# djeday123/kaldi-fp16

Measured on AMD Instinct MI355X. Metric: frames/sec CNN-TDNN fwd+bwd, 40-dim×1500-frame egs, 1/2/4/8 MI355X, higher is better.
Workload: dtype fp16

## Files before the change

### include/kf_ops.h

```cpp
#ifndef KALDI_FP16_AMD_KF_OPS_H
#define KALDI_FP16_AMD_KF_OPS_H

#include <stddef.h>
#include <stdint.h>

#ifdef __cplusplus
extern "C" {
#endif

#define KF_MAX_PARTS 9
#define KF_ZERO 0
#define KF_CLAMP 1

typedef struct {
    const void *base;
    long long ld;
    int nrows, ncols;
    int kcontig;
    int nparts, part_width;
    int T, hout, hsrc, hmul, hdiv, tpolicy;
    int dt[KF_MAX_PARTS];
    int dh[KF_MAX_PARTS];
    int edge_t[KF_MAX_PARTS];
    int edge_row[KF_MAX_PARTS];
// ... 149 lines not shown
                void *scratch);
long long kf_ng_state_scratch_bytes(const KfNgPre *pres, int npre);
int kf_ng_state(const KfNgPre *pres, const KfNgPre *pres_dev, int npre, const KfNgOpts *opts, int update,
                float *w32, void *w16, double *sc, const float *stat, void *scratch, float *report);

#define KF_DROP_MAX 32
typedef struct KfDropLayer {
    float *mask;
    long long ld;
    int dim;
    int ordinal;
    float p;
    int reserved;
} KfDropLayer;
int kf_dropout_masks(int n, const KfDropLayer *layers, int B, unsigned long long seed, long long step);
int kf_row_seg(int32_t *row_seg, const int *dev_seq_off, int B, int T, int tc0, int tc);

int kf_specaug_rows(int32_t *row_band, const int *dev_seq_off, int B, int T, int dim, int max_bins, float z,
                    int max_zeroed, int max_kept, unsigned ordinal, unsigned long long seed, long long step);
int kf_specaug_apply(const void *x, long long ldx, void *y, long long ldy, long long rows, int dim,
                     const int32_t *row_band);

int kf_bn_train_stats(const void *r, long long ld, int rows, int D, float eps, float target_rms, float *mean,
                      float *var, float *scale, float *shift, double *acc_count, double *acc_sum, double *acc_sumsq);
int kf_bn_train_apply(const void *r, long long ld, int rows, int D, const float *scale, const float *shift,
                      const float *drop, long long ld_drop, const int32_t *row_seg, const void *resid, long long ldr,
                      float alpha, void *out, long long ldo);
int kf_bn_train_bwd_stats(const void *g, long long ldg, const void *r, long long ldr, int rows, int D,
                          const float *scale, const float *shift, float target_rms, const float *drop,
                          long long ld_drop, const int32_t *row_seg, float *a, float *b);
int kf_bn_train_bwd_apply(const void *g, long long ldg, const void *r, long long ldr, int rows, int D,
                          const float *scale, const float *shift, float target_rms, const float *a, const float *b,
                          const float *drop, long long ld_drop, const int32_t *row_seg, const uint8_t *mask,
                          long long ld_mask, void *dz, long long lddz);

int kf_gather_rows(void *dst, const void *src, long long row_bytes, int T, int tc0, int tc);
int kf_scatter_rows(void *dst, const void *src, long long row_bytes, int T, int tc0, int tc);
int kf_scatter_rows_from(void *dst, const void *src, long long row_bytes, int T, int tc0, int tc, int r0);
int kf_rows_sum_list(void *edge, const void *src, long long ld, const int *rows, int n, int cols);
const char *kf_layers_last_error(void);

enum { KF_CM_ONEBYTE_COLHDR = 1, KF_CM_TWOBYTE = 2, KF_CM_ONEBYTE = 3, KF_CM_FLOAT = 4 };
typedef struct {
    int format, rows, cols, out_row;
    float min_value, range;
    long long payload_off;
} KfCmDesc;
int kf_cm_expand(const KfCmDesc *dev_desc, int nmat, int max_rows, int max_cols,
                 const void *dev_blob, void *dev_out, int ldo);
int kf_cm_expand_host(const KfCmDesc *desc, int nmat, int max_rows, int max_cols,
                      const void *blob, size_t blob_bytes, void *dev_out, int ldo);

typedef struct {
    const void *proj;
    long long ldp;
    int T, num_heads, key_dim, value_dim, context, num_left, stride;
    float key_scale;
} KfAttention;
int kf_attention_forward(const KfAttention *a, void *out, long long ldo, uint8_t *mask, const float *scale,
                         const float *shift);
int kf_attention_backward(const KfAttention *a, const void *dz, long long ldz, void *dproj, float *scratch);

int kf_combine_feature_maps(const void *a, long long lda, const void *b, long long ldb, const int *dev_seq_off,
                            int B, void *out, long long ldo, int T, int height, int nf1, int nf2);
int kf_combine_feature_maps_backward(const void *dy, long long ldy, const int *dev_seq_off, int B, void *db,
                                     long long ldb, int height, int nf1, int nf2);
int kf_im2col_small(const void *x, long long ldx, int T, int hin, int hout, int sub, int fin, int ntaps,
                    const int *dt, const int *dh, void *P, int kp);
int kf_col2im_small(const void *dP, int T, int hin, int hout, int sub, int fin, int ntaps, const int *dt,
                    const int *dh, int kp, void *dx, long long ldx);
int kf_rows_gemm(const void *x, long long ldx, const void *W, long long ldw, void *y, long long ldy, int R, int K,
                 int N);
int kf_rows_wgrad(const void *x, long long ldx, const void *g, long long ldg, float *dW, long long ldd, int R, int M,
                  int N);
int kf_scale_cols(const void *x, long long ldx, const float *scale, void *y, long long ldy, int rows, int cols);

void kf_prof_enable(int on);
int kf_prof_reserve(int n);
int kf_prof_collect(int cls, long long *count, double *ms, double *flops);
int kf_prof_collect2(int cls, long long *count, double *ms, double *flops, double *bytes);
void kf_prof_reset(void);

void kf_gemm_debug_kil(int on);
#define KF_TRANSPOSE_MAX 48
int kf_transpose_batch(int n, const void *const *src, void *const *dst, const int *M, const int *N);
void kf_halo_trace(unsigned long long *buf, int at);
int kf_halo_debug_last(int *out, int n);
void kf_gemm_trace(unsigned long long *buf, int at, int blk);

const char *kf_last_error(void);
void kf_clear_error(void);
int kf_prof_records(int max, int *cls, float *ms, double *flops, int *mnkt);

int kf_take_pending(const char *where);
const char *kf_pending_log(void);
void kf_pending_clear(void);
int kf_peek_error(void);
int kf_debug_spin(void *stream, long long cycles);

#ifdef __cplusplus
}
#endif
#endif
```

### kaldi-fp16_amd/csrc/conv_halo.hip

```cpp
#include "gemm_kernel.h"

__device__ __forceinline__ int halo_off(int R, int c) {
    return (R >> 3) * 1024 + 256 * (c >> 1) + 16 * ((c + 2 * R) & 15);
}
struct HaloArgs {
    const h16 *x;
    long long ld;
    int T, hout, hmul, hsrc, pw, pad, hpe, hpos, nf, dtmin;
    int ntaps, nch;
    int ts, toff;
    int rows;
    int npieces;
    int slice;
    int halo_bytes;
    int nbuf;
    int ctap[KF_MAX_PARTS];
    int bshift[KF_MAX_PARTS];
    unsigned mhpos;
    unsigned long long *trace;
};


template <int BM, int BN, int WM, int WN, bool BKC, int BMODE, bool BROW, int ST>
__global__ __launch_bounds__(64 * WM * WN, 1) void conv_halo_kernel(int M, int N, OpD B, KfEpilogue E,
                                                                    HaloArgs H, int n_mtiles,
                                                                    int n_ntiles) {
    constexpr int NW = WM * WN;
    constexpr int WTM = BM / WM, WTN = BN / WN;
    constexpr int TM = WTM / 16, TN = WTN / 16;
    constexpr int B_STAGE = BN * BK * 2;
    constexpr int NWB = NW / 2;
    using SB = Stager<BKC, BN, BMODE, NWB>;
    static_assert(SB::EVEN, "uniform B loads per B wave");
    static_assert(ST == 2, "the split-wave waits are written for a two-stage B ring");
    extern __shared__ __attribute__((aligned(16))) char dsm[];
    char *bring = dsm + H.nbuf * H.halo_bytes;

    const int tid = threadIdx.x, lane = tid & 63;
    const int wave = __builtin_amdgcn_readfirstlane(tid >> 6);
    const int wm = wave / WN, wn = wave % WN;

    const int ntiles = n_mtiles * n_ntiles;
    int tile = blockIdx.x;
    if (ntiles >= 8) {
        const int q = ntiles / 8, rmd = ntiles % 8, xcd = tile % 8, loc = tile / 8;
        tile = (xcd < rmd ? xcd * (q + 1) : rmd * (q + 1) + (xcd - rmd) * q) + loc;
    }
    const int mt = tile / n_ntiles, nt = tile - mt * n_ntiles;
    const int m0 = mt * BM, n0 = nt * BN;
    const int tbase = H.ts * (m0 / H.hout) + H.toff + H.dtmin;

    const bool bwave = wave < NWB;
    SB sb;
    if (bwave) sb.init(B, n0, wave, lane);
    const Rsrc rx = make_rsrc(H.x), rb = make_rsrc(B.base);
    const int K = H.ntaps * H.pw;

    auto halo_issue = [&](int c, int img, int q0, int q1, int w0, int nw) {
        char *dst = dsm + img * H.halo_bytes;
        const int slot = lane & 15, kc = 2 * (lane >> 4) + (slot & 1), r = ((slot - kc) & 15) >> 1;
        if (wave < w0) return;
        for (int q = q0 + wave - w0; q < q1; q += nw) {
            const int R = 8 * q + r;
            unsigned voff = BAD;
            if (R < H.rows) {
                const int f = (int)__umulhi((unsigned)R, H.mhpos), pos = R - f * H.hpos;
                const int par = pos >= H.hpe ? 1 : 0, idx = pos - par * H.hpe;
                const int sh = idx * H.hmul + par - H.pad, t = tbase + f;
                if ((unsigned)t < (unsigned)H.T && (unsigned)sh < (unsigned)H.hsrc)
                    voff = (unsigned)(((long long)t * H.ld + (long long)sh * H.pw + c * BK + kc * 8) * 2);
            }
            lds_dma<16>(rx, dst + q * 1024, voff);
        }
    };

    int rb0[TM];
    static_for<TM>([&](auto I) {
        const int r = wm * WTM + I * 16 + (lane & 15);
        const int m = min(m0 + r, M - 1);
        const int t = m / H.hout, h = m - t * H.hout;
        rb0[I] = (H.ts * t + H.toff - tbase + H.dtmin) * H.hpos + h;
    });

    float4v acc[TM][TN];
    static_for<TM>([&](auto I) {
        static_for<TN>([&](auto J) { acc[I][J] = float4v{0.f, 0.f, 0.f, 0.f}; });
    });
// ... 220 lines not shown
```

### kaldi-fp16_amd/csrc/gemm_common.h

```cpp
#pragma once
#include <utility>

#include "kf_common.h"
#include "../../include/kf_ops.h"

struct OpD {
    const h16 *base;
    long long ld;
    int nrows, ncols;
    int nparts, pw;
    int T, hout, hsrc, hmul, hshift;
    int tclamp, simple, p64;
    unsigned inv_hout;
    unsigned ldb, pwb;
    int edges;
    int dt[KF_MAX_PARTS], dh[KF_MAX_PARTS], et[KF_MAX_PARTS], er[KF_MAX_PARTS];
    const uint8_t *sc;
    unsigned lds;
    int pw8;
    const uint8_t *mk;
    unsigned mlim;
    int tmul, t0;
};

#include <utility>
template <typename F, int... Is>
__device__ __forceinline__ void static_for_impl(F &&f, std::integer_sequence<int, Is...>) {
    (f(std::integral_constant<int, Is>{}), ...);
}
template <int N, typename F>
__device__ __forceinline__ void static_for(F &&f) {
    static_for_impl(f, std::make_integer_sequence<int, N>{});
}

template <typename T>
__device__ __forceinline__ T sel9(const T (&a)[KF_MAX_PARTS], int p, int nparts) {
    if (nparts <= 2) return p ? a[1] : a[0];
    T v = a[0];
#pragma unroll
    for (int i = 1; i < KF_MAX_PARTS; ++i)
        if (p == i) v = a[i];
    return v;
}

__device__ __forceinline__ long long op_off(const OpD &d, int t, int h, int kk, int dtp, int dhp,
                                            int etp, int erp) {
    int st;
    if (t == etp) {
        st = erp;
    } else {
        st = t + dtp;
        if (d.tclamp) st = min(max(st, 0), d.T - 1);
        else if ((unsigned)st >= (unsigned)d.T) return -1;
    }
    int sh = h * d.hmul + dhp;
    if (d.hshift) {
        if (sh & ((1 << d.hshift) - 1)) return -1;
        sh >>= d.hshift;
    }
    if ((unsigned)sh >= (unsigned)d.hsrc) return -1;
    return (long long)st * d.ld + (long long)sh * d.pw + kk;
}

constexpr int BK = 64;
__device__ __forceinline__ int kc_off(int r, int c) { return r * 128 + 16 * (c ^ ((r >> 1) & 7)); }
template <int W>
__device__ __forceinline__ int mn_swz(int r) {
    if constexpr (W % 128 == 0) return ((r & 3) << 2) ^ (((r >> 3) & 1) << 4);
    else if constexpr (W % 64 == 0) return ((r & 2) << 1) ^ (((r >> 3) & 1) << 3);
    else if constexpr (W % 32 == 0) return ((r >> 3) & 1) << 2;
    else return 0;
}
template <int W>
__device__ __forceinline__ int mn_off(int r, int u) {
    return r * (W * 2) + 8 * (u ^ mn_swz<W>(r));
}

typedef __attribute__((address_space(3))) short4v lds_s4;
typedef int v4i_t __attribute__((ext_vector_type(4)));

template <bool KC, int W>
__device__ __forceinline__ half8 load_frag(const char *tile, int idx0, int s, int lane) {
    if constexpr (KC) {
        const int r = idx0 + (lane & 15);
        const int c = s * 4 + (lane >> 4);
        return *reinterpret_cast<const half8 *>(tile + kc_off(r, c));
    } else {
        const int q = (lane & 15) >> 2, p = lane & 3, g = lane >> 4;
        const int r0 = s * 32 + 8 * g + q;
        const int u = (idx0 >> 2) + p;
        short4v lo = __builtin_amdgcn_ds_read_tr16_b64_v4i16((lds_s4 *)(tile + mn_off<W>(r0, u)));
        short4v hi =
            __builtin_amdgcn_ds_read_tr16_b64_v4i16((lds_s4 *)(tile + mn_off<W>(r0 + 4, u)));
        typedef short short8v __attribute__((ext_vector_type(8)));
        short8v v = __builtin_shufflevector(lo, hi, 0, 1, 2, 3, 4, 5, 6, 7);
        return __builtin_bit_cast(half8, v);
    }
}

enum { OP_SIMPLE = 0, OP_P2 = 1, OP_GEN = 2 };
constexpr int OP_MASKED = 8;
constexpr int EPI_DROP = 16;
constexpr unsigned BAD = 0xFFFFFFFFu;

typedef unsigned Rsrc __attribute__((ext_vector_type(4)));
__device__ __forceinline__ Rsrc make_rsrc(const void *base) {
    const unsigned long long b = (unsigned long long)base;
    return Rsrc{(unsigned)__builtin_amdgcn_readfirstlane((unsigned)b),
                (unsigned)__builtin_amdgcn_readfirstlane((unsigned)(b >> 32)) & 0xFFFFu, 0xFFFFFFFFu, 0x00020000u};
}

template <int BYTES>
__device__ __forceinline__ void lds_dma(Rsrc rs, const void *lds_dst, unsigned voff) {
    const unsigned m0v = (unsigned)__builtin_amdgcn_readfirstlane((unsigned)(uintptr_t)lds_dst);
    unsigned keep;
    if constexpr (BYTES == 16)
        asm volatile("s_mov_b32 %0, m0\n\ts_mov_b32 m0, %3\n\ts_nop 0\n\tbuffer_load_dwordx4 %1, %2, 0 offen lds\n\t"
                     "s_mov_b32 m0, %0"
                     : "=&s"(keep)
                     : "v"(voff), "s"(rs), "s"(m0v)
                     : "memory");
    else
        asm volatile("s_mov_b32 %0, m0\n\ts_mov_b32 m0, %3\n\ts_nop 0\n\tbuffer_load_dword %1, %2, 0 offen lds\n\t"
                     "s_mov_b32 m0, %0"
                     : "=&s"(keep)
                     : "v"(voff), "s"(rs), "s"(m0v)
                     : "memory");
}

__device__ __forceinline__ unsigned op_boff(const OpD &d, int t, int h, int kk, int dtp, int dhp,
                                            int etp, int erp) {
    const long long off = op_off(d, t, h, kk, dtp, dhp, etp, erp);
    return off < 0 ? BAD : (unsigned)(off * 2);
}

template <bool KC, int TR, int MODE, int NW, bool MK = false>
struct Stager {
    static constexpr int NP = TR / 8;
    static constexpr int NC = (NP + NW - 1) / NW;
    static constexpr bool EVEN = NC * NW == NP;
    static_assert(NP * 8 == TR, "tile rows must be a multiple of 8");
    unsigned o0[NC];
    unsigned o1[MODE == OP_P2 && KC ? NC : 1];
    int th[MODE == OP_GEN ? NC : 1];
    int dt1[!KC && MODE != OP_SIMPLE ? NC : 1];
    unsigned mbv[MK ? NC : 1];
    int curp;

// ... 278 lines not shown
```

### kaldi-fp16_amd/csrc/gemm_fused.hip

```cpp
#include "gemm_fused.h"

static int g_kil = 1;
extern "C" void kf_gemm_debug_kil(int on) { g_kil = on != 0; }

static int fused_impl(int M, int N, int K, const KfOperand *A, const KfOperand *B, const KfEpilogue *epi,
                      const WgradArgs *edge);
extern "C" int kf_gemm_fused(int M, int N, int K, const KfOperand *A, const KfOperand *B,
                             const KfEpilogue *epi) {
    return fused_impl(M, N, K, A, B, epi, nullptr);
}
extern "C" int kf_gemm_fused_edge(int M, int N, int K, const KfOperand *A, const KfOperand *B,
                                  const KfEpilogue *epi, void *edge_out, const void *x0, const void *x1,
                                  const void *W, int cols) {
    if (!edge_out || !x0 || !x1 || !W || cols <= 0 || cols % 8 || ((uintptr_t)x0 | (uintptr_t)x1 | (uintptr_t)W) & 15 ||
        A->fmt != KF_FMT_MXFP8 || M <= 0) {
        kf_report_error("kf_gemm_fused_edge: an MXFP8 product with M > 0, an edge row and 16-byte aligned fp16 "
                        "operands, cols %% 8 == 0 (cols=%d)", cols);
        return -1;
    }
    WgradArgs g{};
    g.eo = (h16 *)edge_out;
    g.ex0 = (const h16 *)x0;
    g.ex1 = (const h16 *)x1;
    g.ew = (const h16 *)W;
// ... 34 lines not shown
        return -1;
    }
    WgradArgs G{nullptr, nullptr, 0, 0, g_kil};
    if (edge) {
        G.eo = edge->eo;
        G.ex0 = edge->ex0;
        G.ex1 = edge->ex1;
        G.ew = edge->ew;
        G.ecols = edge->ecols;
    }
    const int am = op_mode(a), bm = op_mode(b);
    const bool f8 = A->fmt == KF_FMT_MXFP8;
    if (f8 != (B->fmt == KF_FMT_MXFP8)) {
        kf_report_error("kf_gemm_fused: both operands must be MXFP8, or neither");
        return -1;
    }
    if (E.row_group && (f8 || a.mk || b.mk)) {
        kf_report_error("kf_gemm_fused: grouped output rows (row_group) need an fp16 conv input gradient");
        return -1;
    }
    if (E.drop) {
        if (!E.row_seg || (E.scale != nullptr) == (E.out2 != nullptr)) {
            kf_report_error("kf_gemm_fused: drop needs row_seg and exactly one of scale (forward) and out2 (input "
                            "gradient)");
            return -1;
        }
        if (E.row_group || E.out8 || E.beta != 0.f || f8 || a.mk || b.mk || edge || am == OP_GEN || bm == OP_GEN) {
            kf_report_error("kf_gemm_fused: drop does not go with row_group, out8, beta, MXFP8, masked or conv operands");
            return -1;
        }
        if (E.ld_drop < N || E.ld_drop % 8 || ((uintptr_t)E.drop & 15) || ((uintptr_t)E.row_seg & 3)) {
            kf_report_error("kf_gemm_fused: drop needs ld_drop >= N, ld_drop %% 8 == 0 and a 16-byte aligned table "
                            "(ld_drop=%lld N=%d)", E.ld_drop, N);
            return -1;
        }
    }
    if (f8) {
        if (K % 128 || am == OP_GEN || a.edges || bm != OP_SIMPLE) {
            kf_report_error("kf_gemm_fused: MXFP8 needs K %% 128 == 0, a plain or time-spliced A and a "
                            "plain B (K=%d)", K);
            return -1;
        }
        const int K2 = K / 2;
        if (N % 160 == 0 && N <= 320 && !E.out8) {
            if (am == OP_SIMPLE)
                return launch<384, 160, 4, 2, true, true, false, 2, OP_SIMPLE, OP_SIMPLE, 1>(M, N, K2, a, b, E, G, 1);
            return launch<384, 160, 4, 2, true, true, false, 2, OP_P2, OP_SIMPLE, 1>(M, N, K2, a, b, E, G, 1);
        }
        if (N >= 256) {
            if (am == OP_SIMPLE)
                return launch<256, 256, 2, 4, true, true, false, 2, OP_SIMPLE, OP_SIMPLE, 1>(M, N, K2, a, b, E, G, 1);
            return launch<256, 256, 2, 4, true, true, false, 2, OP_P2, OP_SIMPLE, 1>(M, N, K2, a, b, E, G, 1);
        }
        if (am == OP_SIMPLE)
            return launch<128, 128, 2, 2, true, true, false, 2, OP_SIMPLE, OP_SIMPLE, 1>(M, N, K2, a, b, E, G, 1);
        return launch<128, 128, 2, 2, true, true, false, 2, OP_P2, OP_SIMPLE, 1>(M, N, K2, a, b, E, G, 1);
    }
    if (a.mk || b.mk) {
        if (!b.mk && B->kcontig && !E.out8 && ((am == OP_P2 && bm == OP_P2) || (am == OP_SIMPLE && bm == OP_SIMPLE))) {
            const int mt = N % 160 == 0 && N <= 320 ? 5 : N <= 64 ? 2 : 0;
#define KF_MASKED(AM_, BM_)                                                                                    \
    do {                                                                                                       \
        if (mt == 5) return launch<384, 160, 4, 2, true, true, false, 2, AM_ | OP_MASKED, BM_>(M, N, K, a, b, E, G, 1); \
        if (mt == 2) return launch<256, 64, 4, 1, true, true, false, 2, AM_ | OP_MASKED, BM_>(M, N, K, a, b, E, G, 1);  \
        return launch<128, 128, 2, 2, true, true, false, 2, AM_ | OP_MASKED, BM_>(M, N, K, a, b, E, G, 1);               \
    } while (0)
            if (am == OP_P2) KF_MASKED(OP_P2, OP_P2);
            KF_MASKED(OP_SIMPLE, OP_SIMPLE);
#undef KF_MASKED
        }
        kf_report_error("kf_gemm_fused: a masked operand must be A (plain or two-part time splice, with a "
                        "k-contiguous B of the same kind, no MXFP8 copy) (M=%d N=%d K=%d)", M, N, K);
        return -1;
    }
    if (!E.drop) {
        const int hr = conv_halo_try(M, N, K, a, b, bm, B->kcontig != 0, E);
        if (hr != 0) return hr < 0 ? -1 : 0;
    }
    if (a.tmul > 1 || a.t0 || b.tmul > 1 || b.t0 || E.row_group) {
        kf_report_error("kf_gemm_fused: time-strided rows (tmul / t0) and grouped output rows (row_group) need a "
                        "conv on the halo kernel (M=%d N=%d K=%d)", M, N, K);
        return -1;
    }
    int tile = 0;
    if (N % 160 == 0 && N <= 320 && !E.out8) tile = 5;
    else if (N <= 64) tile = 2;
    else if (N >= 256) tile = 6;
    if (tile == 6 && K <= 640 && N % 192 == 0 && !E.out8) tile = 7;
    if (tile == 5 && (long long)((M + 383) / 384) * ((N + 159) / 160) < 192) tile = 8;
    if (!B->kcontig) return fused_mn(tile, am, bm, M, N, K, a, b, E, G);
    if (E.drop) {
        if (am == OP_SIMPLE && bm == OP_SIMPLE) return fused_tile_drop<true, OP_SIMPLE, OP_SIMPLE>(tile, M, N, K, a, b, E, G);
        if (am == OP_P2 && bm == OP_SIMPLE) return fused_tile_drop<true, OP_P2, OP_SIMPLE>(tile, M, N, K, a, b, E, G);
        if (am == OP_P2 && bm == OP_P2) return fused_tile_drop<true, OP_P2, OP_P2>(tile, M, N, K, a, b, E, G);
        kf_report_error("kf_gemm_fused: drop with a plain A needs a plain B (M=%d N=%d K=%d)", M, N, K);
        return -1;
    }
    if (am == OP_SIMPLE && bm == OP_SIMPLE) return fused_tile<true, OP_SIMPLE, OP_SIMPLE>(tile, M, N, K, a, b, E, G);
    if (am == OP_P2 && bm == OP_SIMPLE) return fused_tile<true, OP_P2, OP_SIMPLE>(tile, M, N, K, a, b, E, G);
    if (am == OP_P2 && bm == OP_P2) return fused_tile<true, OP_P2, OP_P2>(tile, M, N, K, a, b, E, G);
    return fused_tile<true, OP_GEN, OP_GEN>(tile, M, N, K, a, b, E, G);
}
```

### kaldi-fp16_amd/csrc/gemm_host.h

```cpp
#pragma once
#include <algorithm>

#include "gemm_common.h"

double kf_gemm_alg_bytes(const OpD &a, const OpD &b, const KfEpilogue &E, long long M, long long N);

int kf_conv_wgrad_halo_try(int M, int N, int K, const OpD &a, const OpD &b, float *dW, long long ldw,
                           float *bias_grad, int accumulate);
constexpr int KF_HALO_DBG_N = 16;
int *kf_halo_dbg_begin(int kind);

void kf_wgrad_reduce(const float *slab, const float *bias_slab, int splits, int M, int N, float *dW,
                     long long ldw, float *bias_grad, int accumulate, const float *cs = nullptr);

#pragma GCC visibility push(hidden)
bool to_dev(const KfOperand &d, OpD &o, const char *name);
double op_src_bytes(const OpD &o, int f8);
double epi_bytes(const KfEpilogue &E, long long M, long long N);
unsigned long long *kf_gemm_trace_take(int *blk);
int conv_halo_try(int M, int N, int K, const OpD &a, const OpD &b, int bm, bool bkc, const KfEpilogue &E);
#pragma GCC visibility pop

static inline int op_mode(const OpD &o) {
    if (o.simple) return OP_SIMPLE;
    if (o.nparts <= 2 && o.hout == 1 && o.hmul == 0 && o.hshift == 0) return OP_P2;
    return OP_GEN;
}
static inline bool mn_gen_ok(const OpD &o, const char *name) {
    if (op_mode(o) == OP_GEN && o.edges) {
        kf_report_error("operand %s: edge rows need a time-only (<= 2 part) reduction-major operand", name);
        return false;
    }
    return true;
}

static inline KfOperand plain_operand(const void *p, long long ld, int rows, int cols, int kcontig) {
    KfOperand d;
    memset(&d, 0, sizeof(d));
    d.base = p;
    d.ld = ld;
    d.nrows = rows;
    d.ncols = cols;
    d.kcontig = kcontig;
    d.nparts = 1;
    d.part_width = cols;
    d.T = rows;
    d.hout = 1;
    d.hsrc = 1;
    d.hmul = 0;
    d.hdiv = 1;
    d.tpolicy = KF_ZERO;
    for (int i = 0; i < KF_MAX_PARTS; ++i) d.edge_t[i] = -1;
    return d;
}

struct TapGeom {
    int dtmin, dtmax;
    int pad;
    int hpe;
};
static inline TapGeom tap_geometry(const OpD &a) {
    int dtmin = 1 << 20, dtmax = -(1 << 20), dhmin = 1 << 20, dhmax = -(1 << 20);
    for (int p = 0; p < a.nparts; ++p) {
        dtmin = std::min(dtmin, a.dt[p]);
        dtmax = std::max(dtmax, a.dt[p]);
        dhmin = std::min(dhmin, a.dh[p]);
        dhmax = std::max(dhmax, a.dh[p]);
    }
    TapGeom g{dtmin, dtmax, std::max(0, -dhmin), 0};
    const int maxshp = (a.hout - 1) * a.hmul + dhmax + g.pad;
    const int HP = std::max(a.hsrc + g.pad, maxshp + 1);
    g.hpe = (HP + a.hmul - 1) / a.hmul;
    return g;
}
static inline void tap_rows(const OpD &a, const TapGeom &g, int hpe, int *ctap) {
    for (int p = 0; p < a.nparts; ++p) {
        const int x = a.dh[p] + g.pad;
        ctap[p] = (a.dt[p] - g.dtmin) * hpe * a.hmul + (x % a.hmul) * hpe + x / a.hmul;
    }
}
```

### kaldi-fp16_amd/python/kfp16/__init__.py

```python
from __future__ import annotations

import ctypes as C
import os

import numpy as np

_HERE = os.path.dirname(os.path.abspath(__file__))
LIBDIR = os.environ.get("KFP16_LIBDIR") or os.path.normpath(os.path.join(_HERE, "..", "..", "lib"))
INCDIR = os.path.normpath(os.path.join(_HERE, "..", "..", "..", "include"))


class KfError(RuntimeError):
    pass


def _load(name):
    path = os.path.join(LIBDIR, name)
    if not os.path.exists(path):
        raise ImportError(
            f"kfp16: {path} is missing — build the HIP libraries first "
            "(python -c 'import __graft_entry__ as g; g.build()'); there is no CPU fallback")
    if os.environ.get("KF_ERR_TRACE", "0") not in ("", "0"):
        return _TracedCDLL(path, mode=C.RTLD_GLOBAL)
    return C.CDLL(path, mode=C.RTLD_GLOBAL)
# ... 206 lines not shown

    def __del__(self):
        try:
            self.free()
        except Exception:
            pass


def upload_fp16(arr: np.ndarray) -> DeviceBuffer:
    a = np.ascontiguousarray(arr, dtype=np.float16)
    buf = DeviceBuffer(a.nbytes)
    check(core.bridge_transfer_fp16(buf.ptr, a.ctypes.data, a.size), "upload_fp16")
    buf.shape = a.shape
    return buf


def upload_f32(arr: np.ndarray) -> DeviceBuffer:
    a = np.ascontiguousarray(arr, dtype=np.float32)
    buf = DeviceBuffer(a.nbytes)
    check(core.bridge_transfer_float32(buf.ptr, a.ctypes.data, a.size), "upload_f32")
    buf.shape = a.shape
    return buf


def read_fp16(ptr, shape) -> np.ndarray:
    out = np.empty(shape, dtype=np.float16)
    check(core.bridge_read_fp16(out.ctypes.data, ptr, out.size), "read_fp16")
    return out


def read_f32(ptr, shape) -> np.ndarray:
    out = np.empty(shape, dtype=np.float32)
    check(core.bridge_read_float32(out.ctypes.data, ptr, out.size), "read_f32")
    return out


def hip_runtimes():
    with open("/proc/self/maps") as f:
        return sorted({l.split()[-1] for l in f if "libamdhip64" in l})


def assert_single_hip_runtime():
    libs = hip_runtimes()
    if len(libs) > 1:
        raise KfError(f"two HIP runtimes loaded {libs}: import torch before kfp16")


def prof_collect(cls: int):
    n, ms, fl = _ll(), C.c_double(), C.c_double()
    core.kf_prof_collect(cls, C.byref(n), C.byref(ms), C.byref(fl))
    return n.value, ms.value, fl.value


def prof_collect2(cls: int):
    n, ms, fl, by = _ll(), C.c_double(), C.c_double(), C.c_double()
    core.kf_prof_collect2(cls, C.byref(n), C.byref(ms), C.byref(fl), C.byref(by))
    return n.value, ms.value, fl.value, by.value


def prof_records(max_n: int = 4096):
    cls = (C.c_int * max_n)()
    ms = (C.c_float * max_n)()
    fl = (C.c_double * max_n)()
    mnkt = (C.c_int * (4 * max_n))()
    n = core.kf_prof_records(max_n, cls, ms, fl, mnkt)
    return [dict(cls=cls[i], ms=ms[i], flops=fl[i], M=mnkt[4 * i], N=mnkt[4 * i + 1], K=mnkt[4 * i + 2],
                 tile=mnkt[4 * i + 3]) for i in range(n)]


def halo_debug_last() -> dict:
    v = (_i * 16)()
    core.kf_halo_debug_last(v, 16)
    if v[0] == 1:
        names = ("BM", "BN", "brow", "nch", "nbuf", "hpe", "hpos", "pad", "mtiles", "ntiles")
    elif v[0] == 2:
        names = ("BN", "waves", "stages", "npieces", "hpw", "splits", "kps")
    else:
        return dict(kind=None, taken=0)
    d = dict(kind="fused" if v[0] == 1 else "wgrad", taken=v[1])
    d.update({k: v[2 + i] for i, k in enumerate(names)})
    return d


def set_stream(stream_handle) -> None:
    core.kf_set_stream(C.c_void_p(stream_handle) if stream_handle else None)


def sync() -> None:
    check(core.bridge_gpu_sync(), "sync")


class Network:

    def __init__(self, xconfig: str, max_frames: int, layout_only: bool = False):
        create = nnet.nnet_create_layout if layout_only else nnet.nnet_create
        self.h = create(xconfig.encode(), int(max_frames))
        if not self.h:
            raise KfError("nnet_create: " + _err(nnet.nnet_last_error))
        self.max_frames = int(max_frames)
        self.layers = []
        name = C.create_string_buffer(256)
        ty, di, do = _i(), _i(), _i()
        for i in range(nnet.nnet_num_layers(self.h)):
            nnet.nnet_layer_info(self.h, i, name, 256, C.byref(ty), C.byref(di), C.byref(do))
            self.layers.append((name.value.decode(), ty.value, di.value, do.value))
        self.num_params = nnet.nnet_num_params(self.h)
        self.params = {}
        r, c, off = _i(), _i(), _ll()
        for i in range(nnet.nnet_num_param_tensors(self.h)):
            nnet.nnet_param_info(self.h, i, name, 256, C.byref(r), C.byref(c), C.byref(off))
            self.params[name.value.decode()] = (r.value, c.value, off.value)
        self.T = 0

    def close(self):
        if getattr(self, "h", None):
            nnet.nnet_free(self.h)
            self.h = None

    def __del__(self):
        try:
            self.close()
        except Exception:
            pass

    def flat_params(self, named: dict) -> np.ndarray:
        flat = np.zeros(self.num_params, dtype=np.float32)
        for k, (r, c, off) in self.params.items():
            flat[off:off + r * c] = np.asarray(named[k], dtype=np.float32).reshape(-1)
        return flat

    def unflatten(self, flat: np.ndarray) -> dict:
        return {k: flat[off:off + r * c].reshape(r, c) for k, (r, c, off) in self.params.items()}

    def set_params(self, named: dict):
        flat = self.flat_params(named)
        check(nnet.nnet_set_params(self.h, flat.ctypes.data), "nnet_set_params")

    def get_params(self) -> dict:
        flat = np.empty(self.num_params, dtype=np.float32)
        check(nnet.nnet_get_params(self.h, flat.ctypes.data), "nnet_get_params")
        return self.unflatten(flat)

    def set_bn(self, layer, which, mean, var, gamma, beta, eps=1e-3, target_rms=None):
        target_rms = 0.0 if target_rms is None else target_rms
        arrs = [np.ascontiguousarray(a, dtype=np.float32) for a in (mean, var, gamma, beta)]
        check(nnet.nnet_set_bn(self.h, layer.encode(), which, *[a.ctypes.data for a in arrs],
                               float(eps), float(target_rms)), "nnet_set_bn")

    def forward(self, features_ptr, T: int):
        check(nnet.nnet_forward(self.h, features_ptr, int(T)), "nnet_forward")
        self.T = int(T)

    def forward_ivector(self, features_ptr, T: int, ivectors_ptr, seq_row0):
        so = np.ascontiguousarray(seq_row0, dtype=np.int32)
        check(nnet.nnet_forward_ivector(self.h, features_ptr, int(T), ivectors_ptr, len(so) - 1,
                                        so.ctypes.data), "nnet_forward_ivector")
        self.T = int(T)

    def activation(self, layer: str):
        r, c = _i(), _i()
        p = nnet.nnet_activation(self.h, layer.encode(), C.byref(r), C.byref(c))
        if not p:
            raise KfError("nnet_activation: " + _err(nnet.nnet_last_error))
        return p, r.value, c.value

    def read_activation(self, layer: str) -> np.ndarray:
# ... 276 lines not shown
              "nnet_bind_dp")


def parse_summary(xconfig: str):
    n = nnet.nnet_parse_summary(xconfig.encode(), None, 0)
    if n < 0:
        raise KfError("nnet_parse_summary: " + _err(nnet.nnet_last_error))
    buf = C.create_string_buffer(n)
    nnet.nnet_parse_summary(xconfig.encode(), buf, n)
    lines = buf.value.decode().strip().splitlines()
    layers = [(a, int(b), int(c), int(d)) for a, b, c, d in (l.split() for l in lines[:-1])]
    return layers, int(lines[-1].split()[1])


def read_header_symbols(header: str):
    import re
    text = open(os.path.join(INCDIR, header)).read()
    text = re.sub(r"/\*.*?\*/", "", text, flags=re.S)
    text = re.sub(r"//[^\n]*", "", text)
    names = re.findall(r"\b([a-z][a-z0-9_]*)\s*\([^;{]*\)\s*;", text)
    return sorted(set(n for n in names if not n.startswith(("sizeof", "typedef"))))


MAXP = 9


class KfOperand(C.Structure):
    _fields_ = [("base", _vp), ("ld", _ll), ("nrows", _i), ("ncols", _i), ("kcontig", _i),
                ("nparts", _i), ("part_width", _i), ("T", _i), ("hout", _i), ("hsrc", _i),
                ("hmul", _i), ("hdiv", _i), ("tpolicy", _i), ("dt", _i * MAXP), ("dh", _i * MAXP),
                ("edge_t", _i * MAXP), ("edge_row", _i * MAXP), ("fmt", _i), ("scales", _vp),
                ("lds", _ll), ("mask", _vp), ("mask_rows", _i), ("tmul", _i), ("t0", _i)]


FMT_FP16, FMT_MXFP8 = 0, 1


class KfEpilogue(C.Structure):
    _fields_ = [("out", _vp), ("ldo", _ll), ("alpha", _f), ("beta", _f), ("bias", _vp), ("relu", _i),
                ("mask_out", _vp), ("scale", _vp), ("shift", _vp), ("resid", _vp), ("ldr", _ll),
                ("resid_alpha", _f), ("out2", _vp), ("ldo2", _ll), ("scale2", _vp), ("mask_in", _vp),
                ("out8", _vp), ("ldo8", _ll), ("scale8", _vp), ("out8_src", _i), ("edge_out", _vp),
                ("edge_r0", _i), ("edge_r1", _i), ("edge_src", _i),
                ("row_group", _i), ("row_stride", _i),
                ("drop", _vp), ("ld_drop", _ll), ("row_seg", _vp)]


def operand(base, ld, rows, cols, kcontig, nparts=1, part_width=None, T=None, hout=1, hsrc=1,
            hmul=0, hdiv=1, tpolicy=0, dt=(), dh=(), edges=(), scales=None, lds=0, mask=None, mask_rows=0):
    o = KfOperand()
    if mask is not None:
        o.mask, o.mask_rows = mask, mask_rows
    if scales is not None:
        o.fmt, o.scales, o.lds = FMT_MXFP8, scales, lds
    o.base, o.ld, o.nrows, o.ncols, o.kcontig = base, ld, rows, cols, kcontig
    o.nparts, o.part_width = nparts, part_width if part_width is not None else cols
    o.T = T if T is not None else rows
    o.hout, o.hsrc, o.hmul, o.hdiv, o.tpolicy = hout, hsrc, hmul, hdiv, tpolicy
    for i in range(MAXP):
        o.edge_t[i] = -1
    for i, v in enumerate(dt):
        o.dt[i] = v
    for i, v in enumerate(dh):
        o.dh[i] = v
    for p, t, row in edges:
        o.edge_t[p] = t
        o.edge_row[p] = row
    return o


_sig(core, "kf_gemm_fused", _i, _i, _i, _i, C.POINTER(KfOperand), C.POINTER(KfOperand), C.POINTER(KfEpilogue))
_sig(core, "kf_gemm_wgrad", _i, _i, _i, _i, C.POINTER(KfOperand), C.POINTER(KfOperand), _vp, _ll, _vp, _i)
_sig(core, "kf_rows_sum", _i, _vp, _vp, _ll, _i, _i, _i)
_sig(core, "kf_rows_sum_mask", _i, _vp, _vp, _ll, _i, _i, _i, _vp)
_sig(core, "kf_dot2_rows", _i, _vp, _vp, _vp, _vp, _i, _i)
_sig(core, "kf_gemm_fused_edge", _i, _i, _i, _i, C.POINTER(KfOperand), C.POINTER(KfOperand), C.POINTER(KfEpilogue),
     _vp, _vp, _vp, _vp, _i)
_sig(core, "kf_scale_cols", _i, _vp, _ll, _vp, _vp, _ll, _i, _i)
_sig(core, "kf_gemm_wgrad_scaled", _i, _i, _i, _i, C.POINTER(KfOperand), C.POINTER(KfOperand), _vp, _ll, _vp, _i,
     _vp)
_sig(core, "kf_gemm_wgrad_target", _i, _i)
_sig(core, "kf_gemm_debug_kil", None, _i)
_sig(core, "kf_gemm_trace", None, _vp, _i, _i)
_sig(core, "kf_halo_debug_last", _i, C.POINTER(_i), _i)
_sig(core, "kf_quant_mxfp8", _i, _vp, _ll, _i, _i, _i, _vp, _ll, _vp, _ll)
_ip = C.POINTER(_i)
_sig(core, "kf_small_gemm", _i, _vp, _i, _vp, _vp, _i, _i, _i, _i)
_sig(core, "kf_bn_apply", _i, _vp, _vp, _ll, _i, _vp, _vp)
_sig(core, "kf_conv_c1_forward", _i, _i, _i, _i, _i, _i, _i, _ip, _ip, _vp, _vp, _vp, _vp, _vp, _vp, _vp)
_sig(core, "kf_conv_c1_wgrad", _i, _i, _i, _i, _i, _i, _i, _ip, _ip, _vp, _vp, _vp, _vp)
_sig(core, "kf_sgd_flat", _i, _vp, _vp, _vp, _vp, _f, _f, _ll)
_sig(core, "kf_f32_to_f16_flat", _i, _vp, _vp, _ll)


class KfUpdSegment(C.Structure):
    _fields_ = [("begin", _ll), ("end", _ll), ("comp", _i), ("first_wg", _i)]


class KfUpdComp(C.Structure):
    _fields_ = [("max_change", _f), ("l2", _f), ("lr_factor", _f), ("first_wg", _i), ("num_wg", _i)]


UPD_CHUNK = 4096
_sig(core, "kf_update_scratch_bytes", _ll, _ll, _i, _i)
_sig(core, "kf_update_maxchange", _i, _vp, _vp, _vp, _vp, _ll, _vp, _i, _vp, _i, _f, _f, _f, _f, _vp, _vp)


class KfOrthoMat(C.Structure):
    _fields_ = [("offset", _ll), ("K", _i), ("n", _i), ("c", _f), ("reserved", _i)]


_sig(core, "kf_orthonormal_scratch_bytes", _ll, _vp, _i)
_sig(core, "kf_orthonormal_constrain", _i, _vp, _vp, _ll, _vp, _vp, _i, _vp, _vp)


class KfNgOpts(C.Structure):
    _fields_ = [("rank_in", _i), ("rank_out", _i), ("update_period", _i), ("num_samples_history", _f),
                ("alpha", _f), ("epsilon", _f), ("delta", _f)]


class KfNgPre(C.Structure):
    _fields_ = [("D", _i), ("R", _i), ("w_off", _ll), ("h_off", _ll), ("s_off", _ll), ("st_off", _ll)]


class KfNgComp(C.Structure):
    _fields_ = [("dw_off", _ll), ("db_off", _ll), ("K", _i), ("N", _i), ("pre_in", _i), ("pre_out", _i)]


NG_MAX_RANK, NG_REPORT = 96, 8


def ng_rp(R: int) -> int:
    return (R + 31) // 32 * 32


def ng_w16_ld(D: int) -> int:
    return (D + 7) // 8 * 8


def ng_stat_offsets(D: int, R: int) -> dict:
    Rp = ng_rp(R)
    return dict(L=32, JT=32 + Rp * Rp, floats=32 + Rp * Rp + D * Rp)


_sig(core, "kf_ng_default_opts", None, C.POINTER(KfNgOpts))
_sig(core, "kf_ng_init", _i, _vp, _vp, _i, C.POINTER(KfNgOpts), _vp, _vp, _vp)
_sig(core, "kf_ng_trx", _i, C.POINTER(KfOperand), _i, _vp)
_sig(core, "kf_ng_scales", _i, _vp, _vp, _i, C.POINTER(KfNgOpts), _vp, _vp, _vp)
_sig(core, "kf_ng_apply_scratch_bytes", _ll, _vp, _i, _vp, _i)
_sig(core, "kf_ng_apply", _i, _vp, _ll, _vp, _vp, _i, _vp, _vp, _i, _vp, _vp, _vp)
_sig(core, "kf_ng_state_scratch_bytes", _ll, _vp, _i)
_sig(core, "kf_ng_state", _i, _vp, _vp, _i, C.POINTER(KfNgOpts), _i, _vp, _vp, _vp, _vp, _vp, _vp)
class KfDropLayer(C.Structure):
    _fields_ = [("mask", _vp), ("ld", _ll), ("dim", _i), ("ordinal", _i), ("p", _f), ("reserved", _i)]


_sig(core, "kf_dropout_masks", _i, _i, _vp, _i, C.c_uint64, _ll)
_sig(core, "kf_row_seg", _i, _vp, _vp, _i, _i, _i, _i)
_sig(core, "kf_bn_train_stats", _i, _vp, _ll, _i, _i, _f, _f, _vp, _vp, _vp, _vp, _vp, _vp, _vp)
_sig(core, "kf_bn_train_apply", _i, _vp, _ll, _i, _i, _vp, _vp, _vp, _ll, _vp, _vp, _ll, _f, _vp, _ll)
_sig(core, "kf_bn_train_bwd_stats", _i, _vp, _ll, _vp, _ll, _i, _i, _vp, _vp, _f, _vp, _ll, _vp, _vp, _vp)
_sig(core, "kf_bn_train_bwd_apply", _i, _vp, _ll, _vp, _ll, _i, _i, _vp, _vp, _f, _vp, _vp, _vp, _ll, _vp, _vp, _ll,
     _vp, _ll)
_sig(core, "kf_specaug_rows", _i, _vp, _vp, _i, _i, _i, _i, _f, _i, _i, C.c_uint, C.c_uint64, _ll)
_sig(core, "kf_specaug_apply", _i, _vp, _ll, _vp, _ll, _ll, _i, _vp)
_sig(core, "kf_gather_rows", _i, _vp, _vp, _ll, _i, _i, _i)
# ... 11 lines not shown
```

Measured before the change: 3.880 million.

## Add splice-once GEMM kernel that loads each TDNN input row once for both taps

Adds a specialised fp16 GEMM path for two-part spliced TDNN operands (N of 160 or 320). Each block DMAs a contiguous image of the input rows covering both time offsets into LDS once per K chunk, then reads both taps' A fragments from that shared image instead of gathering each part separately. The goal is to cut redundant global loads of overlapping spliced rows, with a multi-buffered image pipeline overlapping the B-stage loads. It is enabled by default only when the grid is small, and it adds a large new kernel with edge-row and zero-row handling that could be slower or wrong on corner cases.

```diff
diff --git a/include/kf_ops.h b/include/kf_ops.h
--- a/include/kf_ops.h
+++ b/include/kf_ops.h
@@ -255,6 +255,10 @@
 void kf_prof_reset(void);
 
 void kf_gemm_debug_kil(int on);
+void kf_gemm_debug_splice_once(int on);
+int kf_splice_once_debug_plan(int M, int N, int K, const KfOperand *A, const KfOperand *B,
+                              const KfEpilogue *epi, int *out, int n);
+int kf_splice_once_debug_last(int *out, int n);
 #define KF_TRANSPOSE_MAX 48
 int kf_transpose_batch(int n, const void *const *src, void *const *dst, const int *M, const int *N);
 void kf_halo_trace(unsigned long long *buf, int at);
diff --git a/kaldi-fp16_amd/csrc/conv_halo.hip b/kaldi-fp16_amd/csrc/conv_halo.hip
--- a/kaldi-fp16_amd/csrc/conv_halo.hip
+++ b/kaldi-fp16_amd/csrc/conv_halo.hip
@@ -1,8 +1,5 @@
 #include "gemm_kernel.h"
 
-__device__ __forceinline__ int halo_off(int R, int c) {
-    return (R >> 3) * 1024 + 256 * (c >> 1) + 16 * ((c + 2 * R) & 15);
-}
 struct HaloArgs {
     const h16 *x;
     long long ld;
diff --git a/kaldi-fp16_amd/csrc/gemm_common.h b/kaldi-fp16_amd/csrc/gemm_common.h
--- a/kaldi-fp16_amd/csrc/gemm_common.h
+++ b/kaldi-fp16_amd/csrc/gemm_common.h
@@ -64,6 +64,9 @@
 
 constexpr int BK = 64;
 __device__ __forceinline__ int kc_off(int r, int c) { return r * 128 + 16 * (c ^ ((r >> 1) & 7)); }
+__device__ __forceinline__ int halo_off(int R, int c) {
+    return (R >> 3) * 1024 + 256 * (c >> 1) + 16 * ((c + 2 * R) & 15);
+}
 template <int W>
 __device__ __forceinline__ int mn_swz(int r) {
     if constexpr (W % 128 == 0) return ((r & 3) << 2) ^ (((r >> 3) & 1) << 4);
diff --git a/kaldi-fp16_amd/csrc/gemm_fused.hip b/kaldi-fp16_amd/csrc/gemm_fused.hip
--- a/kaldi-fp16_amd/csrc/gemm_fused.hip
+++ b/kaldi-fp16_amd/csrc/gemm_fused.hip
@@ -140,6 +140,10 @@
                         "conv on the halo kernel (M=%d N=%d K=%d)", M, N, K);
         return -1;
     }
+    if (!f8) {
+        const int sr = splice_once_try(M, N, K, a, b, B->kcontig != 0, E);
+        if (sr != 0) return sr < 0 ? -1 : 0;
+    }
     int tile = 0;
     if (N % 160 == 0 && N <= 320 && !E.out8) tile = 5;
     else if (N <= 64) tile = 2;
diff --git a/kaldi-fp16_amd/csrc/gemm_host.h b/kaldi-fp16_amd/csrc/gemm_host.h
--- a/kaldi-fp16_amd/csrc/gemm_host.h
+++ b/kaldi-fp16_amd/csrc/gemm_host.h
@@ -19,6 +19,7 @@
 double epi_bytes(const KfEpilogue &E, long long M, long long N);
 unsigned long long *kf_gemm_trace_take(int *blk);
 int conv_halo_try(int M, int N, int K, const OpD &a, const OpD &b, int bm, bool bkc, const KfEpilogue &E);
+int splice_once_try(int M, int N, int K, const OpD &a, const OpD &b, bool bkc, const KfEpilogue &E);
 #pragma GCC visibility pop
 
 static inline int op_mode(const OpD &o) {
diff --git a/kaldi-fp16_amd/csrc/splice_once.hip b/kaldi-fp16_amd/csrc/splice_once.hip
--- /dev/null
+++ b/kaldi-fp16_amd/csrc/splice_once.hip
@@ -0,0 +1,304 @@
+#include "gemm_kernel.h"
+
+constexpr int SPL_MAX_PIECES = 20;
+struct SpliceArgs {
+    const h16 *x;
+    unsigned ldb;
+    int T, tclamp, pw;
+    int dt[2], et[2], er[2];
+    int eslot[2];
+    int lo;
+    int nspan;
+    int zrow;
+    int npieces;
+    int img_bytes, nimg, nch;
+    unsigned long long *trace;
+    int trace_blk;
+};
+
+__device__ __forceinline__ void wait_vmcnt_img(int n) {
+    switch (n) {
+        case 1: wait_vmcnt<1>(); break;
+        case 2: wait_vmcnt<2>(); break;
+        case 3: wait_vmcnt<3>(); break;
+        case 4: wait_vmcnt<4>(); break;
+        case 5: wait_vmcnt<5>(); break;
+        default: wait_vmcnt<0>(); break;
+    }
+}
+
+template <int BN, bool BKC, int BMODE, int STB, int WM>
+__global__ __launch_bounds__(128 * WM, 1) void splice_once_kernel(int M, int N, int K, OpD B, KfEpilogue E,
+                                                                  SpliceArgs S, int n_mtiles, int n_ntiles) {
+    constexpr int BM = 128, WN = 2, NW = WM * WN;
+    constexpr int WTM = BM / WM, WTN = BN / WN;
+    constexpr int TM = WTM / 16, TN = WTN / 16;
+    static_assert(TN * 16 == WTN && TM * 16 == WTM, "wave tile multiple of 16");
+    constexpr int B_STAGE = BN * BK * 2;
+    using SB = Stager<BKC, BN, BMODE, NW>;
+    static_assert(STB == 4, "two B stages of two slabs (a chunk's part-0 and part-1 slab) each");
+    constexpr int MAXQ = (SPL_MAX_PIECES + NW - 1) / NW;
+    extern __shared__ __attribute__((aligned(16))) char dsm[];
+    char *const bring = dsm + S.nimg * S.img_bytes;
+
+    const int tid = threadIdx.x, lane = tid & 63;
+    const int wave = __builtin_amdgcn_readfirstlane(tid >> 6);
+    const int wm = wave / WN, wn = wave % WN;
+    const int bid = blockIdx.x;
+    const bool trb = S.trace != nullptr && tid == 0, trp = trb && bid == S.trace_blk;
+    if (trb) {
+        S.trace[64 + 3 * bid] = wall_clock64();
+        S.trace[64 + 3 * bid + 2] = (unsigned long long)__builtin_amdgcn_s_getreg((4) | (31 << 11)) |
+                                    ((unsigned long long)__builtin_amdgcn_s_getreg((20) | (31 << 11)) << 32);
+    }
+#define SPL_TP(slot) \
+    if (trp) S.trace[slot] = wall_clock64();
+    SPL_TP(0);
+    if (trb && bid == 0) {
+        S.trace[60] = (unsigned long long)M | ((unsigned long long)N << 20) | ((unsigned long long)K << 40);
+        S.trace[61] = (unsigned long long)BM | ((unsigned long long)BN << 16) | ((unsigned long long)gridDim.x << 32);
+        S.trace[62] = 1;
+    }
+
+    const int ntiles = n_mtiles * n_ntiles;
+    int tile = blockIdx.x;
+    if (ntiles >= 8) {
+        const int q = ntiles / 8, rmd = ntiles % 8, xcd = tile % 8, loc = tile / 8;
+        tile = (xcd < rmd ? xcd * (q + 1) : rmd * (q + 1) + (xcd - rmd) * q) + loc;
+    }
+    const int mt = tile / n_ntiles, nt = tile - mt * n_ntiles;
+    const int m0 = mt * BM, n0 = nt * BN;
+
+    SB sb;
+    sb.init(B, n0, wave, lane);
+    const Rsrc rx = make_rsrc(S.x), rb = make_rsrc(B.base);
+
+    unsigned aoff[MAXQ];
+    {
+        const int slot = lane & 15, kc = 2 * (lane >> 4) + (slot & 1), r = ((slot - kc) & 15) >> 1;
+        const int src0 = m0 + S.lo;
+        static_for<MAXQ>([&](auto Q) {
+            const int R = 8 * (wave + decltype(Q)::value * NW) + r;
+            unsigned ro = BAD;
+            if (R < S.nspan) {
+                int st = src0 + R;
+                if (S.tclamp) st = min(max(st, 0), S.T - 1);
+                if ((unsigned)st < (unsigned)S.T) ro = (unsigned)st * S.ldb;
+            } else if (R != S.zrow) {
+#pragma unroll
+                for (int p = 0; p < 2; ++p)
+                    if (R == S.eslot[p] && S.et[p] >= m0 && S.et[p] < min(m0 + BM, M)) ro = (unsigned)S.er[p] * S.ldb;
+            }
+            aoff[decltype(Q)::value] = ro == BAD ? BAD : ro + (unsigned)(kc * 16);
+        });
+    }
+    int na = 0;
+#pragma unroll
+    for (int j = 0; j < MAXQ; ++j) na += wave + j * NW < S.npieces;
+    auto img_issue = [&](int c, int img) {
+        char *dst = dsm + img * S.img_bytes;
+        const unsigned cb = (unsigned)(c * BK * 2);
+        static_for<MAXQ>([&](auto Q) {
+            const int q = wave + decltype(Q)::value * NW;
+            const unsigned o = aoff[decltype(Q)::value];
+            if (q < S.npieces) lds_dma<16>(rx, dst + q * 1024, o == BAD ? BAD : o + cb);
+        });
+    };
+
+    int ri[2][TM];
+    static_for<TM>([&](auto I) {
+        const int r = wm * WTM + I * 16 + (lane & 15), m = m0 + r;
+#pragma unroll
+        for (int p = 0; p < 2; ++p) {
+            int R = S.zrow;
+            if (m < M) {
+                const int st = m + S.dt[p];
+                if (m == S.et[p]) R = S.eslot[p];
+                else if (S.tclamp || (unsigned)st < (unsigned)S.T) R = r + S.dt[p] - S.lo;
+            }
+            ri[p][I] = R;
+        }
+    });
+
+    float4v acc[TM][TN];
+    static_for<TM>([&](auto I) {
+        static_for<TN>([&](auto J) { acc[I][J] = float4v{0.f, 0.f, 0.f, 0.f}; });
+    });
+    const EpiPre epre = epi_params<BN, 64 * NW>(E, N, n0, tid);
+
+    const int nch = S.nch;
+    for (int c = 0; c < S.nimg - 1 && c < nch; ++c) img_issue(c, c);
+    if (nch > 0) {
+        sb.issue(B, rb, 0, K, bring, wave, lane);
+        sb.issue(B, rb, S.pw, K, bring + B_STAGE, wave, lane);
+    }
+    SPL_TP(1);
+    int ia = 0, ib = 0;
+    int after = 0;
+    for (int c = 0; c < nch; ++c) {
+        wait_vmcnt_img(after);
+        __builtin_amdgcn_s_barrier();
+        __builtin_amdgcn_sched_barrier(0);
+        if (c < 40) SPL_TP(2 + c);
+        after = 0;
+        if (c + 1 < nch) {
+            char *dst = bring + (ib ^ 1) * (2 * B_STAGE);
+            sb.issue(B, rb, (c + 1) * BK, K, dst, wave, lane);
+            sb.issue(B, rb, S.pw + (c + 1) * BK, K, dst + B_STAGE, wave, lane);
+            if (c + S.nimg - 1 < nch) {
+                img_issue(c + S.nimg - 1, ia ? ia - 1 : S.nimg - 1);
+                after = na;
+            }
+        }
+        const char *ta = dsm + ia * S.img_bytes;
+        static_for<2>([&](auto P) {
+            constexpr int p = decltype(P)::value;
+            const char *tb = bring + ib * (2 * B_STAGE) + p * B_STAGE;
+            static_for<BK / 32>([&](auto SS) {
+                constexpr int s = decltype(SS)::value;
+                half8 fa[TM], fb[TN];
+                static_for<TM>([&](auto I) {
+                    fa[I] = *reinterpret_cast<const half8 *>(ta + halo_off(ri[p][I], s * 4 + (lane >> 4)));
+                });
+                static_for<TN>([&](auto J) { fb[J] = load_frag<BKC, BN>(tb, wn * WTN + J * 16, s, lane); });
+                static_for<TM>([&](auto I) {
+                    static_for<TN>([&](auto J) {
+                        acc[I][J] = __builtin_amdgcn_mfma_f32_16x16x32_f16(fa[I], fb[J], acc[I][J], 0, 0, 0);
+                    });
+                });
+            });
+        });
+        __builtin_amdgcn_sched_barrier(0);
+        ib ^= 1;
+        ia = ia + 1 == S.nimg ? 0 : ia + 1;
+    }
+    SPL_TP(42);
+    fused_epilogue<BM, BN, WM, WN>(acc, dsm, E, M, N, m0, n0, tid, lane, wave, &epre);
+    SPL_TP(43);
+    if (trb) S.trace[64 + 3 * bid + 1] = wall_clock64();
+#undef SPL_TP
+}
+
+static int g_splice_once = 1;
+extern "C" void kf_gemm_debug_splice_once(int on) { g_splice_once = on < 0 ? 0 : on > 2 ? 1 : on; }
+
+constexpr int SPL_STB = 4;
+constexpr int SPL_WM = 4;
+struct SplicePlan {
+    SpliceArgs S;
+    size_t lds;
+    bool bkc;
+    int span, nedge, rows;
+};
+
+constexpr int KF_SPL_DBG_N = 16;
+static thread_local int g_spl_dbg[KF_SPL_DBG_N];
+
+static bool splice_once_plan(int M, int N, int K, const OpD &a, const OpD &b, bool bkc, bool f8,
+                             const KfEpilogue &E, SplicePlan &P) {
+    memset(&P, 0, sizeof P);
+    if (f8 || a.mk || b.mk || E.drop || E.out8 || E.row_group) return false;
+    if (N != 160 && N != 320) return false;
+    if (op_mode(a) != OP_P2 || a.nparts != 2 || a.pw % BK || a.pw < 8 * BK || K != 2 * a.pw || a.ncols != K) return false;
+    if (a.dh[0] || a.dh[1] || a.hsrc < 1 || a.T < 1 || a.tmul != 1 || a.t0) return false;
+    if (std::abs(a.dt[0]) > 8 || std::abs(a.dt[1]) > 8) return false;
+    if (bkc ? op_mode(b) != OP_P2 : op_mode(b) != OP_SIMPLE) return false;
+    if (b.tmul != 1 || b.t0) return false;
+    SpliceArgs &S = P.S;
+    S.x = a.base;
+    S.ldb = a.ldb;
+    S.T = a.T;
+    S.tclamp = a.tclamp;
+    S.pw = a.pw;
+    S.lo = std::min(a.dt[0], a.dt[1]);
+    P.span = std::max(a.dt[0], a.dt[1]) - S.lo;
+    S.nspan = 128 + P.span;
+    for (int p = 0; p < 2; ++p) {
+        S.dt[p] = a.dt[p];
+        S.et[p] = a.et[p];
+        S.er[p] = a.er[p];
+        S.eslot[p] = S.nspan + P.nedge;
+        if (a.et[p] >= 0) ++P.nedge;
+    }
+    S.zrow = S.nspan + P.nedge;
+    P.rows = S.zrow + 1;
+    S.npieces = (P.rows + 7) / 8;
+    if (S.npieces > SPL_MAX_PIECES) return false;
+    S.img_bytes = S.npieces * 1024;
+    S.nch = a.pw / BK;
+    P.bkc = bkc;
+    const size_t epi = 16 * 160 + 32 * EpiMap<80>::LDT * 4 * 2 * SPL_WM;
+    for (S.nimg = 4; S.nimg >= 3; --S.nimg) {
+        P.lds = std::max((size_t)S.nimg * S.img_bytes + (size_t)SPL_STB * 160 * BK * 2, epi);
+        if (P.lds <= 160 * 1024) return true;
+    }
+    return false;
+}
+
+static void splice_dbg_fill(int *v, bool applies, int M, int N, const SplicePlan &P) {
+    memset(v, 0, sizeof(int) * KF_SPL_DBG_N);
+    v[0] = 1;
+    v[1] = applies;
+    if (!applies) return;
+    const int f[] = {128, 160, P.span, P.nedge, 1, P.rows, P.S.npieces, P.S.nimg, SPL_STB, (int)P.lds,
+                     (M + 127) / 128, (N + 159) / 160, P.bkc};
+    std::copy(f, f + sizeof f / sizeof f[0], v + 2);
+}
+extern "C" int kf_splice_once_debug_last(int *out, int n) {
+    const int m = std::min(std::max(n, 0), KF_SPL_DBG_N);
+    for (int i = 0; out && i < m; ++i) out[i] = g_spl_dbg[i];
+    return out ? m : 0;
+}
+extern "C" int kf_splice_once_debug_plan(int M, int N, int K, const KfOperand *A, const KfOperand *B,
+                                         const KfEpilogue *epi, int *out, int n) {
+    OpD a, b;
+    if (!A || !B || !epi || !to_dev(*A, a, "A") || !to_dev(*B, b, "B")) return -1;
+    SplicePlan P;
+    const bool ok = A->kcontig && (A->fmt == KF_FMT_MXFP8) == (B->fmt == KF_FMT_MXFP8) &&
+                    splice_once_plan(M, N, K, a, b, B->kcontig != 0, A->fmt == KF_FMT_MXFP8, *epi, P);
+    int v[KF_SPL_DBG_N];
+    splice_dbg_fill(v, ok, M, N, P);
+    const int m = std::min(std::max(n, 0), KF_SPL_DBG_N);
+    for (int i = 0; out && i < m; ++i) out[i] = v[i];
+    return out ? m : 0;
+}
+
+template <bool BKC, int BMODE>
+static int launch_splice(int M, int N, int K, const OpD &a, const OpD &b, const KfEpilogue &E, const SplicePlan &P) {
+    kf_take_pending(__func__);
+    constexpr int BM = 128, BN = 160;
+    const int mt = (M + BM - 1) / BM, nt = (N + BN - 1) / BN;
+    SpliceArgs S = P.S;
+    S.trace = kf_gemm_trace_take(&S.trace_blk);
+    KfProfRec rec{};
+    rec.cls = KF_PROF_FUSED;
+    rec.flops = 2.0 * M * N * (double)K;
+    rec.m = M;
+    rec.n = N;
+    rec.k = K;
+    rec.tile = BM * 10000 + BN;
+    rec.bytes = kf_gemm_alg_bytes(a, b, E, M, N);
+    kf_launch(splice_once_kernel<BN, BKC, BMODE, SPL_STB, SPL_WM>, dim3(mt * nt), dim3(128 * SPL_WM), P.lds, &rec, M, N, K, b, E, S, mt,
+              nt);
+    hipError_t e = hipGetLastError();
+    if (e != hipSuccess) {
+        kf_report_error("splice-once launch (M=%d N=%d K=%d): %s", M, N, K, hipGetErrorString(e));
+        return -1;
+    }
+    if (E.edge_out && E.edge_r0 < E.edge_r1 &&
+        (E.edge_r0 / BM != (E.edge_r1 - 1) / BM || E.edge_r1 > M || E.edge_r0 < 0))
+        return kf_rows_sum_mask(E.edge_out, E.edge_src ? E.out2 : E.out, E.edge_src ? E.ldo2 : E.ldo, E.edge_r0,
+                                E.edge_r1, N, nullptr) < 0 ? -1 : 1;
+    return 1;
+}
+
+int splice_once_try(int M, int N, int K, const OpD &a, const OpD &b, bool bkc, const KfEpilogue &E) {
+    SplicePlan P;
+    bool ok = splice_once_plan(M, N, K, a, b, bkc, false, E, P);
+    const long long grid = (long long)((M + 127) / 128) * ((N + 159) / 160);
+    ok = ok && g_splice_once &&
+         (g_splice_once == 2 || ((long long)((M + 383) / 384) * ((N + 159) / 160) < 192 && grid <= 256));
+    splice_dbg_fill(g_spl_dbg, ok, M, N, P);
+    if (!ok) return 0;
+    return bkc ? launch_splice<true, OP_P2>(M, N, K, a, b, E, P) : launch_splice<false, OP_SIMPLE>(M, N, K, a, b, E, P);
+}
diff --git a/kaldi-fp16_amd/python/kfp16/__init__.py b/kaldi-fp16_amd/python/kfp16/__init__.py
--- a/kaldi-fp16_amd/python/kfp16/__init__.py
+++ b/kaldi-fp16_amd/python/kfp16/__init__.py
@@ -312,6 +312,29 @@
     return d
 
 
+_SPLICE_FIELDS = ("BM", "BN", "span", "edge_slots", "zero_slots", "image_rows", "npieces", "nimg", "b_stages",
+                  "lds", "mtiles", "ntiles", "bkc")
+
+
+def _splice_record(v) -> dict:
+    d = dict(taken=v[1])
+    d.update({k: v[2 + i] for i, k in enumerate(_SPLICE_FIELDS)})
+    return d
+
+
+def splice_once_plan(M, N, K, A, B, E) -> dict:
+    v = (_i * 16)()
+    if core.kf_splice_once_debug_plan(M, N, K, C.byref(A), C.byref(B), C.byref(E), v, 16) < 0:
+        raise KfError("kf_splice_once_debug_plan: " + _err(core.kf_last_error))
+    return _splice_record(v)
+
+
+def splice_once_last() -> dict:
+    v = (_i * 16)()
+    core.kf_splice_once_debug_last(v, 16)
+    return _splice_record(v)
+
+
 def set_stream(stream_handle) -> None:
     core.kf_set_stream(C.c_void_p(stream_handle) if stream_handle else None)
 
@@ -754,6 +777,10 @@
 _sig(core, "kf_gemm_wgrad_target", _i, _i)
 _sig(core, "kf_gemm_debug_kil", None, _i)
 _sig(core, "kf_gemm_trace", None, _vp, _i, _i)
+_sig(core, "kf_gemm_debug_splice_once", None, _i)
+_sig(core, "kf_splice_once_debug_plan", _i, _i, _i, _i, C.POINTER(KfOperand), C.POINTER(KfOperand),
+     C.POINTER(KfEpilogue), C.POINTER(_i), _i)
+_sig(core, "kf_splice_once_debug_last", _i, C.POINTER(_i), _i)
 _sig(core, "kf_halo_debug_last", _i, C.POINTER(_i), _i)
 _sig(core, "kf_quant_mxfp8", _i, _vp, _ll, _i, _i, _i, _vp, _ll, _vp, _ll)
 _ip = C.POINTER(_i)
```

Measured after the change: 3.960 million, median of 6. 1.02x the previous value.
